# markods/GpuSeqAlign

Measured on AMD Instinct MI355X. Metric: GCUPS (DP cell updates/s) + peak HBM GB/s, NW-LG N×M fill, 1/2/4/8 MI355X, higher is better.
Workload: dtype int32; 1 GPU; BASELINE configs[2]: NW-LG 99899x100000 related pair, sparse tile-header (mlsp) fill, tileBx 256 x tileBy 1024, headers only in HBM; R=99899, C=100000, pairs_per_rank=1, representation=sparse tile headers (mlsp), parallelism=pair-sharded x1

## Files before the change

gpuseqalign_amd/__init__.py:

```python
from __future__ import annotations

import ctypes
import dataclasses
import os
from typing import Callable, Dict, Optional, Sequence, Tuple

import numpy as np

__all__ = [
    "NwStat", "NwError", "lib", "Engine", "AlignResult", "SparseResult", "PairDev",
    "NwAlgorithm", "get_nw_algorithm_map", "hash_full", "trace_full", "trace_sparse", "hash_sparse",
    "sparse_align_cost", "sparse_tile_by", "KNOB_NAMES", "LAUNCH_KINDS",
]

_PKG = os.path.dirname(os.path.abspath(__file__))
_SO = os.environ.get("GSA_LIB") or os.path.join(_PKG, "libgsa.so")
_LIB = None


class NwStat:
    success = 0
    helpMenuRequested = 1
    errorCudaGeneral = 2
    errorMemoryAllocation = 3
# ... 42 lines not shown
    def as_dict(self):
        return {"checked": int(self.checked), "mismatches": int(self.mismatches), "first": int(self.first)}


class MemStats(ctypes.Structure):
    _fields_ = [("glmem_peak_allocs", ctypes.c_int64), ("shmem_peak_allocs", ctypes.c_int64),
                ("locmem_peak_allocs", ctypes.c_int64), ("regmem_peak_allocs", ctypes.c_int64)]

    def as_dict(self):
        return {k: int(getattr(self, k)) for k, _ in self._fields_}


class FullTiming(ctypes.Structure):
    _fields_ = [("pass1_ms", ctypes.c_float), ("pass2_ms", ctypes.c_float),
                ("clock_ghz_median", ctypes.c_float), ("clock_ghz_mean", ctypes.c_float),
                ("workgroups", ctypes.c_int64), ("fused", ctypes.c_int32), ("groups", ctypes.c_int32)]


class LaunchInfo(ctypes.Structure):
    _fields_ = [("kind", ctypes.c_int32), ("ns", ctypes.c_int32), ("k", ctypes.c_int32), ("q8", ctypes.c_int32),
                ("q8_declined", ctypes.c_int32), ("staged", ctypes.c_int32), ("mlsppt", ctypes.c_int32),
                ("both_ends", ctypes.c_int32), ("npairs", ctypes.c_int32), ("pair_major", ctypes.c_int32),
                ("trace_band", ctypes.c_int32),
                ("tickets", ctypes.c_int64), ("band_tiles", ctypes.c_int64)]


LAUNCH_KINDS = ("none", "full_lane", "full_fused", "full_two_launch", "sparse_krow", "sparse_strip", "score_krow",
                "score_strip", "score_scan", "trace_sparse", "score_lanes")


class ScoreResult(ctypes.Structure):
    _fields_ = [("score", ctypes.c_int32), ("i_end", ctypes.c_int64), ("j_end", ctypes.c_int64),
                ("calc_kernel_ms", ctypes.c_float)]


class AlignDbResult(ctypes.Structure):
    _fields_ = [("score", ctypes.c_int32), ("status", ctypes.c_int32), ("i_start", ctypes.c_int64),
                ("j_start", ctypes.c_int64), ("i_end", ctypes.c_int64), ("j_end", ctypes.c_int64),
                ("cigar_off", ctypes.c_int64), ("cigar_len", ctypes.c_int64)]


class AlignDbInfo(ctypes.Structure):
    _fields_ = [("lane_hits", ctypes.c_int32), ("unsupported", ctypes.c_int32), ("chunks", ctypes.c_int32),
                ("tasks", ctypes.c_int64), ("code_bytes", ctypes.c_int64), ("fill_ms", ctypes.c_float),
                ("walk_ms", ctypes.c_float)]


# ... 1312 lines not shown
```

gpuseqalign_amd/csrc/gsa_capi.hip:

```cpp
#include <hip/hip_runtime.h>

#include <algorithm>
#include <chrono>
#include <cstdio>
#include <cstdlib>
#include <cstring>
#include <map>
#include <new>
#include <string>
#include <thread>
#include <vector>

#include "../../include/gsa.h"
#include "gsa_ctx.h"
#include "nw_check.h"
#include "nw_lane.h"
#include "nw_expand.h"
#include "nw_krow.h"
#include "nw_strip.h"
#include "nw_trace_dev.h"

namespace gsa {
int fold_moves(const unsigned char* moves, int64_t n, char* edit, int64_t cap, int64_t* edit_len, uint32_t* trace_hash);
}
// ... 13 lines not shown
namespace {

constexpr const char* kKnobNames[] = {
    "GSA_SPARSE_KERNEL", "GSA_KROW_K",      "GSA_KROW_NS",      "GSA_KROW_Q8",       "GSA_LANE_NS",
    "GSA_LANE_FEED",     "GSA_LANE_PAIR",   "GSA_FULL_KERNEL",  "GSA_FULL_FUSED",    "GSA_FULL_SPLIT",
    "GSA_FUSED_STAGED",
    "GSA_EXPAND_RR",     "GSA_BATCH_ORDER", "GSA_SCORE_SCAN",   "GSA_SCORE_KERNEL",  "GSA_SCORE_K",
    "GSA_SCORE_BIDI",    "GSA_SCORE_BIDI_SW", "GSA_BIDI_GRAN",  "GSA_BIDI_SKEW",     "GSA_BIDI_SW_CONT",
    "GSA_BIDI_LOG",      "GSA_TRACE_BAND",  "GSA_TRACE_BAND_BUDGET", "GSA_STAMPS",     "GSA_DB_LANES",
    "GSA_DB_MAXC"};

bool knob_known(const char* name)
{
    for (const char* k : kKnobNames)
        if (std::strcmp(k, name) == 0) return true;
    return false;
}

enum SparseKern { kSpStrip, kSpKrow };
SparseKern sparse_kernel(const gsa_ctx* ctx)
{
    const char* e = knob(ctx, "GSA_SPARSE_KERNEL");
    return (e && std::strcmp(e, "strip") == 0) ? kSpStrip : kSpKrow;
}



int lane_ns(const gsa_ctx* ctx)
{
    const char* e = knob(ctx, "GSA_LANE_NS");
    const int v = e ? std::atoi(e) : gsa::kLaneNSDefault;
    return ((v >= 1 && v <= 4) || v == 6 || v == 8) ? v : gsa::kLaneNSDefault;
}

int run_check(gsa_ctx* ctx, gsa::CheckArgs& a, bool sparse, hipStream_t st, gsa_check_result* out)
{
    hipError_t e = hipSetDevice(ctx->device);
    if (e != hipSuccess) return fail(ctx, e, GSA_ERROR_CUDA_GENERAL);
    int s = reserve_hard(ctx, ctx->buf[kBufChk], 64);
    if (s != GSA_SUCCESS) return s;
    unsigned long long* const chk = ctx->buf[kBufChk].as<unsigned long long>();
    const unsigned long long init[3] = {0ull, 0ull, ~0ull};
    unsigned long long res[3];
    if ((e = hipMemcpyAsync(chk, init, sizeof(init), hipMemcpyHostToDevice, st)) != hipSuccess)
        return fail(ctx, e, GSA_ERROR_MEMORY_TRANSFER);
    a.res = chk;
// ... 93 lines not shown
    for (int p = 0; p < npairs; ++p)
        tileRows += std::max<long long>(1, ((long long)pairs[p].adjrows - 1 + gsa::kSparseTileBy - 1) / gsa::kSparseTileBy);
    const bool fitsChip = tileRows <= (long long)std::max(1, ctx->cu_count);
    const int nsDefault = (npairs > 1 && !fitsChip) ? gsa::kKrowNSBatchDefault : gsa::kKrowNSDefault;
    int krowK = env_int(ctx, "GSA_KROW_K", gsa::kKrowKDefault), krowNS = env_int(ctx, "GSA_KROW_NS", nsDefault);
    if (rows64)
    {
        krowK = 4;
        krowNS = fused ? fused->ns : env_int(ctx, "GSA_KROW_NS", (npairs > 1 && !fitsChip) ? 8 : 4) == 8 ? 8 : 4;
    }
    if (!gsa::krow_ok(krowNS, krowK) || (done && gsa::krow_ticket_rows(krowNS, krowK) != gsa::kSparseTileBy))
    {
        krowK = gsa::kKrowKDefault;
        krowNS = gsa::kKrowNSDefault;
    }
    a.ns = lane ? lane_ns(ctx) : krow ? krowNS : gsa::kSparseNS;
    if (krow && env_int(ctx, "GSA_KROW_Q8", 1) != 0)
    {
        const size_t lds8 = fused ? gsa::full_fused_lds_bytes(krowNS, substsz, true, fused->staged)
                                  : gsa::krow_lds_bytes(krowNS, krowNS == 2 ? 512 : 1024, substsz, true);
        a.q8 = lds8 <= (size_t)ctx->lds_max ? 1 : 0;
    }
    a.q8flag = ctx->ctl + 2;
    const int fullRows = gsa::kLaneRows * a.ns;
    if (mode == gsa::kModeSparse)
    {
        if (tileBx < 64 || tileBx % 16 != 0) return GSA_ERROR_INVALID_VALUE;
        a.tBx = tileBx;
        a.tBy = gsa::kSparseTileBy;
    }
    std::vector<gsa::PairDesc> hd((size_t)npairs);
    long long tickets = 0, gran = 0, maxWork = 1, span = 1;
    for (int p = 0; p < npairs; ++p)
    {
        const gsa_pair_dev& in = pairs[p];
        if (in.adjrows < 1 || in.adjcols < 1 || !in.seqY || !in.seqX) return GSA_ERROR_INVALID_VALUE;
        gsa::PairDesc& d = hd[(size_t)p];
        std::memset(&d, 0, sizeof(d));
        d.seqY = in.seqY;
        d.seqX = in.seqX;
        d.R = in.adjrows - 1;
        d.C = in.adjcols - 1;
        if (mode == gsa::kModeFull)
        {
            if (!in.score) return GSA_ERROR_INVALID_VALUE;
            d.score = in.score;
// ... 32 lines not shown
        tickets += d.nTickets;
        gran += (long long)d.nTickets * gsa::gran_stride(d.Cp);
        if (tickets > (1ll << 30)) return GSA_ERROR_INVALID_VALUE;
    }
    const std::vector<int> sched = batch_schedule(ctx, hd, tickets);
    hipError_t e;
    int s = stage_descs(ctx, hd, sched, st);
    if (s != GSA_SUCCESS) return s;

    gsa::PairDesc* const ddesc = ctx->buf[kBufDesc].as<gsa::PairDesc>();
    a.pairs = ddesc;
    a.nPairs = npairs;
    a.nTicketsTotal = (int)tickets;
    a.sched = sched.empty() ? nullptr : (const int*)(ddesc + npairs);
    a.qcap = (int)(0x7fffffffll / span);
    e = gsa::launch_headers(a, mode, maxWork, st);
    if (e != hipSuccess) return fail(ctx, e, GSA_ERROR_KERNEL_FAILURE);
    auto record = [&](unsigned epoch) {
        gsa_launch_info& li = new_launch_info(
            ctx, lane ? GSA_LAUNCH_FULL_LANE : krow ? GSA_LAUNCH_SPARSE_KROW : GSA_LAUNCH_SPARSE_STRIP, st, epoch);
        li.ns = a.ns;
        li.k = krow ? krowK : 1;
        li.q8 = a.q8;
        li.mlsppt = done ? 1 : 0;
        li.npairs = npairs;
        li.pair_major = (npairs > 1 && sched.empty()) ? 1 : 0;
        li.tickets = tickets;
    };
    if (tickets == 0)
    {
        record(0);
        return GSA_SUCCESS;
    }

    if ((s = ensure_gran(ctx, (size_t)gran, st)) != GSA_SUCCESS) return s;
    a.gran = ctx->buf[kBufGran].as<unsigned long long>();
    a.ticket = ctx->ctl;
    a.err = ctx->ctl + 1;
    a.spin = ctx->spin_ticks;
    a.done = done;
    a.ptChunk = std::max(1, ptChunk);
    a.epoch = ++ctx->epoch;
    if (a.epoch == 0) a.epoch = ++ctx->epoch;
    if (fused)
    {
        if (!rows64) return GSA_ERROR_INVALID_VALUE;
// ... 9 lines not shown
            a.xP = fused->p1;
            a.xrole = ctx->ctl + 4;
            a.xcounter = ctx->ctl + 5;
            if ((e = hipMemsetAsync(a.xrole, 0, 8, st)) != hipSuccess) return fail(ctx, e, GSA_ERROR_MEMORY_TRANSFER);
            ctx->stamps_n = 0;
            if (env_int(ctx, "GSA_STAMPS", 0) &&
                (s = reserve_stamps(ctx, 4 * words + 3 * (size_t)a.xTasks, st, &a.stamps)) != GSA_SUCCESS)
                return s;
        }
        a.xdone = ctx->buf[kBufXdone].as<unsigned long long>();
    }
    if (!fused && krow && !lane && env_int(ctx, "GSA_STAMPS", 0))
    {
        if ((s = reserve_stamps(ctx, 10 * (size_t)tickets * (size_t)krowNS, st, &a.stamps)) != GSA_SUCCESS) return s;
    }
    e = hipMemsetAsync(ctx->ctl, 0, 4, st);
    if (e != hipSuccess) return fail(ctx, e, GSA_ERROR_MEMORY_TRANSFER);
    int grid = (npairs == 1) ? std::max(1, std::min((int)tickets, ctx->cu_count)) : 0;
    a.laneFeed = knob(ctx, "GSA_LANE_FEED") ? env_int(ctx, "GSA_LANE_FEED", 0) : -1;
    a.lanePair = knob(ctx, "GSA_LANE_PAIR") ? env_int(ctx, "GSA_LANE_PAIR", 0) : -1;
    e = lane     ? gsa::launch_lane_fill(a, a.ns, grid, st)
        : fused  ? gsa::launch_full_fused(a, fused->ns, fused->waves, fused->staged, 0, st)
        : rows64 ? gsa::launch_krow_fill_xr(a, krowNS, grid, st)
        : krow   ? gsa::launch_krow_fill(a, krowNS, krowK, 0, grid, st)
                 : gsa::launch_strip_fill(a, mode, grid, st);
    if (e != hipSuccess) return fail(ctx, e, GSA_ERROR_KERNEL_FAILURE);
    note_launch(ctx);
    record(a.epoch);
    return GSA_SUCCESS;
}

int enqueue_fill(gsa_ctx* ctx, int mode, const int32_t* seqY, int32_t adjrows, const int32_t* seqX, int32_t adjcols,
                 const int32_t* subst, int32_t substsz, int32_t gapo, int32_t* score, int32_t tileBx, int32_t* hrow,
                 int32_t* hcol, hipStream_t st, unsigned long long* done = nullptr, int ptChunk = 0,
                 const int32_t* ld = nullptr)
{
    gsa_pair_dev p {seqY, adjrows, seqX, adjcols, score, hrow, hcol};
    return enqueue_batch(ctx, mode, 1, &p, subst, substsz, gapo, tileBx, st, done, ptChunk, ld);
}

constexpr int kNoScratch = -1000;

struct TwoPassOpts
{
    int slot = 0;
    hipEvent_t afterP1 = nullptr, beforeP1 = nullptr, timeP1 = nullptr, startEv = nullptr;
    bool split = false;
// ... 1488 lines not shown
```

gpuseqalign_amd/csrc/nw_krow.h:

```cpp
#pragma once
#include <hip/hip_runtime.h>
#include <stddef.h>

#include "nw_strip.h"

namespace gsa {

constexpr int kKrowKDefault = 4;
constexpr int kKrowNSDefault = 4;
constexpr int kKrowNSBatchDefault = 8;

__host__ __device__ constexpr bool krow_ok(int ns, int k)
{
    return ((k == 2 || k == 4) && (ns == 2 || ns == 4)) || (k == 4 && ns == 8);
}
__host__ __device__ constexpr int krow_ticket_rows(int ns, int k) { return ns * 64 * k; }
__host__ __device__ constexpr int krow_tickets(int trows, int ns, int k)
{
    return (trows * kSparseTileBy + krow_ticket_rows(ns, k) - 1) / krow_ticket_rows(ns, k);
}
size_t krow_lds_bytes(int ns, int lw, int substsz, bool q8 = false);
hipError_t launch_krow_fill(const StripArgs& a, int ns, int k, int lw, int grid, hipStream_t stream);
hipError_t launch_krow_fill_xr(const StripArgs& a, int ns, int grid, hipStream_t stream);
size_t full_fused_lds_bytes(int ns, int substsz, bool q8, bool staged);
hipError_t launch_full_fused(const StripArgs& a, int ns, int waves, bool staged, int grid, hipStream_t stream);

size_t krow_score_lds_bytes(int substsz, bool q8 = false);
hipError_t launch_krow_score(const StripArgs& a, int mode, int k, int grid, hipStream_t stream);
hipError_t launch_krow_score_affine(const StripArgs& a, int mode, int k, int grid, hipStream_t stream);
hipError_t launch_krow_score_semi(const StripArgs& a, int mode, int k, int grid, hipStream_t stream);
hipError_t launch_semi_rowmax(const int* rowR, int R, int C, int go, int ge, int* score, int* jend, hipStream_t stream);
hipError_t launch_krow_score_overlap(const StripArgs& a, int mode, int k, int grid, hipStream_t stream);
hipError_t launch_overlap_max(const int* rowR, const int* colC, int R, int C, int go, int ge, int* res, hipStream_t stream);
hipError_t launch_krow_score_semi_batch(const StripArgs& a, int mode, int k, int grid, hipStream_t stream);
hipError_t launch_semi_rowmax_batch(const PairDesc* pairs, int nPairs, int go, int ge, const unsigned* err, ScoreOut* out,
                                    hipStream_t stream);
hipError_t launch_krow_score_overlap_batch(const StripArgs& a, int mode, int k, int grid, hipStream_t stream);
hipError_t launch_overlap_max_batch(const PairDesc* pairs, int nPairs, int go, int ge, const unsigned* err, ScoreOut* out,
                                    hipStream_t stream);

}
```

gpuseqalign_amd/csrc/nw_krow.hip:

```cpp
#ifndef GSA_PROBE_P1
#define GSA_PROBE_P1 0
#endif
#ifndef GSA_FX_VMCNT
#define GSA_FX_VMCNT 16
#endif
#include <hip/hip_runtime.h>
#include <stdint.h>

#include <algorithm>

#include "nw_expand.h"
#include "nw_krow.h"
#ifdef GSA_KROW_XR
#include "nw_expand_dev.h"
#endif

namespace gsa {
namespace {

__host__ __device__ constexpr int kr_qrs(int lw, bool q8 = false) { return (q8 ? lw / 4 : lw / 2) + 32; }
__host__ __device__ constexpr uint32_t kr_copy1(int lw, int substsz, bool q8 = false)
{
    return (uint32_t)substsz * kr_qrs(lw, q8) + (q8 ? 8u : 16u);
}
// ... 2 lines not shown
    return q8 ? 4u * kr_copy1(lw, substsz, true) : kr_copy1(lw, substsz) + (uint32_t)substsz * kr_qrs(lw) + 16u;
}
constexpr int kBlk = 16;
constexpr int kHalo = kBlk / 4;
constexpr int kRing = 512;
constexpr int kBig = 0x3fffffff;
constexpr int kSubRow = 36;
constexpr int kBatch = 128;
__host__ __device__ constexpr uint32_t kr_prog(int i) { return 8u * (uint32_t)i; }
__host__ __device__ constexpr uint32_t kr_cons(int i) { return 8u * (uint32_t)(i + 1) + 4u; }
constexpr uint32_t kFXo = 4, kFTicket = 132;
constexpr uint32_t kFCap = 160;
constexpr int kXD = 32;
constexpr int kLedgerWords = 10;
#ifndef GSA_KR_BLOCK_LEDGER
#define GSA_KR_BLOCK_LEDGER 0
#endif
#ifndef GSA_KR_LEDGER
#define GSA_KR_LEDGER GSA_KR_BLOCK_LEDGER
#endif
__host__ __device__ constexpr uint32_t kr_xwords(uint32_t flags) { return flags + 256u; }
__host__ __device__ constexpr uint32_t kr_xdata(uint32_t flags) { return flags + 256u + 64u; }
[[maybe_unused]] __host__ __device__ constexpr uint32_t kr_xstage_bytes(int ns) { return 64u + (uint32_t)ns * kXD * 256u; }

extern __shared__ __attribute__((aligned(16))) char krsm[];


typedef int int4v __attribute__((ext_vector_type(4)));
typedef int int2v __attribute__((ext_vector_type(2)));
template <typename T>
using gptr = __attribute__((address_space(1))) T*;
template <typename T>
__device__ __forceinline__ gptr<T> G(T* p)
{
    return (gptr<T>)p;
}

__device__ __forceinline__ int lds_ld(uint32_t a) { return *(const int*)(krsm + a); }
__device__ __forceinline__ void lds_st(uint32_t a, int v) { *(int*)(krsm + a) = v; }
__device__ __forceinline__ int4v lds_ld4(uint32_t a) { return *(const int4v*)(krsm + a); }
__device__ __forceinline__ int raw_ld(uint32_t a)
{
    return __hip_atomic_load((int*)__builtin_assume_aligned(krsm + a, 4), __ATOMIC_RELAXED, __HIP_MEMORY_SCOPE_WORKGROUP);
}
__device__ __forceinline__ int flag_ld(uint32_t a) { return __builtin_amdgcn_readfirstlane(raw_ld(a)); }
__device__ __forceinline__ void flag_st(uint32_t a, int v)
// ... 17 lines not shown
{
    int r;
    asm("v_cndmask_b32_e64 %0, %1, %2, %3" : "=v"(r) : "v"(a), "v"(b), "s"(m));
    return r;
}
__device__ __forceinline__ int qlo(int v) { return (int)(short)v; }
__device__ __forceinline__ int qhi(int v) { return v >> 16; }

struct KrLds
{
    uint32_t q, sub, ring, flags;
};

__host__ __device__ inline KrLds kr_layout(int ns, int lw, int substsz, bool q8 = false)
{
    KrLds L;
    L.q = 0;
    L.sub = kr_qdwords(lw, substsz, q8) * 4u;
    L.ring = L.sub + (uint32_t)substsz * kSubRow * 4u;
    L.flags = L.ring + (uint32_t)(ns + 1) * kRing * 4u;
    return L;
}

template <int NS, int K, int LW, int PT, bool Q8>
__device__ __forceinline__ void kr_strip(const StripArgs& a, const KrLds& L, int tk, int w, int lane)
{
    const int g = a.g;
    const int Cp = a.Cp;
    const int tBx = a.tBx, tBy = a.tBy, tcols = a.tcols;
    const int r0 = tk * (64 * K * NS) + 64 * K * w + 1;
    const int rl = r0 + K * lane;
    constexpr int kLW = LW, kQRS = kr_qrs(LW, Q8);
    constexpr int kQW = Q8 ? kLW / 4 : kLW / 2;
    constexpr int kQD = Q8 ? 4 : 8;
    uint32_t qrow[K];
#pragma unroll
    for (int k = 0; k < K; ++k)
    {
        const int r = rl + k;
        int y = (r <= a.R) ? G(a.seqY)[r] : 0;
        y = ((unsigned)y < (unsigned)a.substsz) ? y : 0;
        qrow[k] = L.q + 4u * ((uint32_t)(lane & (Q8 ? 3 : 1)) * kr_copy1(LW, a.substsz, Q8) + (uint32_t)y * kQRS);
    }
    const uint32_t ring_in = L.ring + (uint32_t)w * (kRing * 4u);
    const uint32_t ring_out = L.ring + (uint32_t)(w + 1) * (kRing * 4u);
    const uint32_t rbase = lane == 0 ? ring_in : ring_out;
    uint32_t roff = lane == 0 ? 4u * 64u : 0u;
    const uint32_t f_in = L.flags + kr_prog(w), f_out = L.flags + kr_prog(w + 1);
    const uint32_t c_out = L.flags + kr_cons(w + 1);
// ... 163 lines not shown
                "ds_write_b128 %7, %10 offset:32\n"
                "ds_write_b128 %7, %11 offset:48\n"
                "s_mov_b64 exec, 1\n"
                "ds_write_b32 %12, %13\n"
                "s_mov_b64 exec, %4\n"
                "s_waitcnt lgkmcnt(5)"
                : "+v"(hc[0]), "+v"(hc[1]), "+v"(hc[2]), "+v"(hc[3]), "=&s"(sv)
                : "v"(hb), "s"(K == 4 ? 0x8000800080008000ull : 0x8000000080000000ull), "v"(sa),
                  "v"(int4v {lt[0], lt[1], lt[2], lt[3]}), "v"(int4v {lt[4], lt[5], lt[6], lt[7]}),
                  "v"(int4v {lt[8], lt[9], lt[10], lt[11]}), "v"(int4v {lt[12], lt[13], lt[14], lt[15]}),
                  "v"(xsWords + 4u * (uint32_t)w), "v"(b)
                : "memory");
        }
        else
            halo_load(b);
    };
    int rpin = 0, rpco = 0, rpxo = 0;
    int rsink = 0;
    const int xoAdd = (w == 0) ? 64 + kBlk - 2 * kBlk : kBig;
    int nbb = tBx / kBlk, jb = 1;
    constexpr bool pt = PT == 1;
    constexpr bool fx = PT >= 3;
    int ptPend = 0;

    auto block = [&](int b, int (&qc)[K][kQD], int (&qn)[K][kQD], auto rampT, bool cap) {
        constexpr bool RAMP = decltype(rampT)::value;
        constexpr bool CAP = !RAMP;
#if GSA_KR_BLOCK_LEDGER
        const uint64_t lt0 = GSA_LDG_T();
        if (ldgEnd) ldg[3] += lt0 - ldgEnd;
#endif
        {
            const int slack = __builtin_amdgcn_readfirstlane(min(min(rpin, rpco + (64 + kRing)), rpxo + xoAdd));
            asm volatile("" ::"v"(rpin), "v"(rpco), "v"(rpxo), "v"(rsink));
            if (slack < kBlk * b + 64 + kBlk && !spin(b)) return false;
        }
        if (PT == 3 && b > 0)
            halo_stage(b);
        else
            halo_load(b);
#if GSA_KR_BLOCK_LEDGER
        const uint64_t lt1 = GSA_LDG_T();
#endif
        const uint32_t pn = q_off(b + 1);
        int va[CAP ? K : 1][CAP ? kBlk : 1];
#pragma unroll
        for (int u = 0; u < kBlk; ++u)
        {
            int nh[K];
            const int up = shr1z(H[K - 1]) + hc[u >> 2][u & 3];
            nh[0] = max3i(D + qv(qc, 0, u), up, H[0]);
#pragma unroll
            for (int k = 1; k < K; ++k) nh[k] = max3i(H[k - 1] + qv(qc, k, u), nh[k - 1], H[k]);
            if constexpr (RAMP)
            {
                const bool border = lane >= kBlk * b + u;
#pragma unroll
                for (int k = 0; k < K; ++k) nh[k] = border ? 0 : nh[k];
            }
            if (u < kQD)
#pragma unroll
                for (int k = 0; k < K; ++k) qn[k][u] = lds_ld(qrow[k] + pn + 4u * u);
            lt[u] = H[K - 1];
            D = up;
#pragma unroll
            for (int k = 0; k < K; ++k)
            {
                H[k] = nh[k];
                if constexpr (CAP) va[k][u] = nh[k];
            }
            if (u == kBlk - 2)
            {
                asm volatile("" ::: "memory");
                const int2v lo = *(const int2v*)(krsm + f_in), hi = *(const int2v*)(krsm + f_in + 16u);
                asm volatile("" ::: "memory");
                rpin = lo.x;
                rpxo = lo.y;
                rpco = hi.y;
                rsink = hi.x;
            }
        }
#if GSA_KR_BLOCK_LEDGER
        const uint64_t lt2 = GSA_LDG_T();
#endif
        handoff(b);
        roff = (roff + 4u * kBlk) & (4u * kRing - 1);
        if constexpr (PT == 4 && !RAMP)
            if ((b & 15) == 15)
            {
                asm volatile("s_waitcnt vmcnt(16)" ::: "memory");
                if (lane == 0)
                    __hip_atomic_store(a.xdone + (size_t)tk * NS + w,
                                       ((unsigned long long)a.epoch << 32) | (unsigned)max(0, kBlk * (b - 7)),
                                       __ATOMIC_RELAXED, __HIP_MEMORY_SCOPE_AGENT);
            }
        if constexpr (PT == 3 && !RAMP)
            if ((b & 15) == 15)
            {
                asm volatile("s_waitcnt vmcnt(%0)" ::"n"(8 * K) : "memory");
                flag_st(xsWords + 4u * (uint32_t)(2 * NS + w), max(0, kBlk * (b + 1) - 2 * tBx - 64));
                const uint64_t t0 = __builtin_amdgcn_s_memrealtime();
                for (unsigned it = 1; flag_ld(xsWords + 4u * (uint32_t)(NS + w)) + kXD < b + 1 + 16; ++it)
                {
                    __builtin_amdgcn_s_sleep(1);
                    if (__builtin_amdgcn_s_memrealtime() - t0 > a.spin || ((it & 31) == 0 && err_set(a)))
                    {
                        atomicOr(a.err, 1u);
                        return false;
                    }
                }
            }
        if (CAP && cap)
        {
            if (pt && ptPend)
            {
                asm volatile("s_waitcnt vmcnt(0)" ::: "memory");
                flag_st(L.flags + kFCap + 4u * (uint32_t)w, ptPend);
                ptPend = 0;
            }
            constexpr uint64_t m1 = 0xAAAAAAAAAAAAAAAAull, m2 = 0xCCCCCCCCCCCCCCCCull;
            constexpr uint64_t m4 = 0xF0F0F0F0F0F0F0F0ull, m8 = 0xFF00FF00FF00FF00ull;
            int v[K];
#pragma unroll
            for (int k = 0; k < K; ++k)
            {
                int x[8];
#pragma unroll
                for (int i = 0; i < 8; ++i) x[i] = sel(m1, va[k][2 * i], va[k][2 * i + 1]);
#pragma unroll
                for (int i = 0; i < 4; ++i) x[i] = sel(m2, x[2 * i], x[2 * i + 1]);
#pragma unroll
                for (int i = 0; i < 2; ++i) x[i] = sel(m4, x[2 * i], x[2 * i + 1]);
                v[k] = sel(m8, x[0], x[1]);
            }
            const int gb = (rl + kBlk * nbb) * g;
// ... 663 lines not shown
                                           __HIP_MEMORY_SCOPE_AGENT);
                    pub[w] = x;
                    moved = true;
                }
                all = all && pub[w] == (int)kXDone;
            }
            if (all) return;
        }
        const uint64_t now = __builtin_amdgcn_s_memrealtime();
        if (moved)
            last = now;
        else
        {
            if (now - last > 4 * a.spin || ((idle & 63) == 0 && err_set(a)))
            {
                atomicOr(a.err, 1u);
                return;
            }
            __builtin_amdgcn_s_sleep(1);
        }
    }
}

__device__ __forceinline__ PairDesc kr_desc(const PairDesc* p)
{
    constexpr int N = sizeof(PairDesc) / 4;
    const int* wds = (const int*)p;
    union
    {
        int v[N];
        PairDesc d;
    } u;
#pragma unroll
    for (int k = 0; k < N; ++k) u.v[k] = __builtin_amdgcn_readfirstlane(G(wds)[k]);
    return u.d;
}

template <int NS, int PT = 0>
constexpr bool kr_split() { return NS <= 4; }
template <int NS, int PT = 0>
constexpr int kr_waves() { return NS + 2 + (kr_split<NS, PT>() ? 1 : 0); }

template <int NS, int K, int LW, int PT, bool Q8>
__global__ void __launch_bounds__((64 * kr_waves<NS, PT>()), 1) nw_krow_kernel(StripArgs a)
{
    const int w = __builtin_amdgcn_readfirstlane(threadIdx.x >> 6);
// ... 75 lines not shown
        else if (kr_split<NS, PT>() && w == NS + 2)
            kr_loader<NS, K, LW, 2, Q8>(pa, L, tk, lane);
        else
        {
            unsigned long long* const lg = (GSA_KR_LEDGER && a.stamps) ? a.stamps + kLedgerWords * ((size_t)tkg * NS + w) : nullptr;
            pa.stamps = lg ? a.stamps + kLedgerWords * (size_t)tkg * NS : nullptr;
            if (lg && lane == 0)
            {
                lg[0] = __builtin_amdgcn_s_memrealtime();
                lg[2] = __builtin_amdgcn_s_memtime();
            }
            __builtin_amdgcn_s_setprio(3);
            kr_strip<NS, K, LW, PT, Q8>(pa, L, tk, w, lane);
            __builtin_amdgcn_s_setprio(0);
            if (lg && lane == 0)
            {
                lg[1] = __builtin_amdgcn_s_memrealtime();
                lg[3] = __builtin_amdgcn_s_memtime();
            }
        }
    }
}

template <int NS, int K, int LW, int PT, bool Q8>
hipError_t launch_kr1(const StripArgs& a, int grid, hipStream_t stream, bool foot = true)
{
    const size_t lds = krow_lds_bytes(NS, LW, a.substsz, Q8);
    auto kern = nw_krow_kernel<NS, K, LW, PT, Q8>;
    hipError_t e = hipFuncSetAttribute((const void*)kern, hipFuncAttributeMaxDynamicSharedMemorySize, (int)lds);
    if (e != hipSuccess) return e;
    if (grid <= 0)
    {
        int per_cu = 0, dev = 0, cus = 0;
        e = hipOccupancyMaxActiveBlocksPerMultiprocessor(&per_cu, (const void*)kern, 64 * kr_waves<NS, PT>(), lds);
        if (e == hipSuccess) e = hipGetDevice(&dev);
        if (e == hipSuccess) e = hipDeviceGetAttribute(&cus, hipDeviceAttributeMultiprocessorCount, dev);
        if (e != hipSuccess) return e;
        grid = std::max(1, std::min(a.nTicketsTotal, std::max(1, per_cu) * cus));
    }
    if (foot && (e = record_foot((const void*)kern, lds, 64 * kr_waves<NS, PT>(), grid)) != hipSuccess) return e;
    hipLaunchKernelGGL(kern, dim3(grid), dim3(64 * kr_waves<NS, PT>()), lds, stream, a);
    return hipGetLastError();
}

template <int NS, int K, int LW, int PT = 0>
hipError_t launch_kr(const StripArgs& a, int grid, hipStream_t stream)
{
    if (!a.q8) return launch_kr1<NS, K, LW, PT, false>(a, grid, stream);
    hipError_t e = launch_kr1<NS, K, LW, PT, true>(a, grid, stream);
    if (e != hipSuccess) return e;
    StripArgs b = a;
    b.q8 = 2;
    return launch_kr1<NS, K, LW, PT, false>(b, grid, stream, false);
}

#ifdef GSA_KROW_SCORE
constexpr int kNegS = -(1 << 29);
typedef int int4u __attribute__((ext_vector_type(4), aligned(4)));
typedef int int2u __attribute__((ext_vector_type(2), aligned(4)));
__device__ __forceinline__ int ks_sel(int a, int b, uint64_t m)
{
    int r;
    asm("v_cndmask_b32_e64 %0, %1, %2, %3" : "=v"(r) : "v"(a), "v"(b), "s"(m));
    return r;
}
__device__ __forceinline__ void ks_sel0(int (&r)[2], const int (&a)[2], const int (&b)[2], int x)
{
    asm("v_cmp_eq_u32 vcc, 0, %6\n\tv_cndmask_b32 %0, %2, %4, vcc\n\tv_cndmask_b32 %1, %3, %5, vcc"
        : "=&v"(r[0]), "=&v"(r[1])
        : "v"(a[0]), "v"(a[1]), "v"(b[0]), "v"(b[1]), "v"(x)
        : "vcc");
}
__device__ __forceinline__ void ks_sel0(int (&r)[4], const int (&a)[4], const int (&b)[4], int x)
{
    asm("v_cmp_eq_u32 vcc, 0, %12\n\tv_cndmask_b32 %0, %4, %8, vcc\n\tv_cndmask_b32 %1, %5, %9, vcc\n\t"
        "v_cndmask_b32 %2, %6, %10, vcc\n\tv_cndmask_b32 %3, %7, %11, vcc"
// ... 1345 lines not shown
{
    if (!a.q8) return launch_fused1<NS, W, false, PTF>(a, grid, stream, true);
    hipError_t e = launch_fused1<NS, W, true, PTF>(a, grid, stream, true);
    if (e != hipSuccess) return e;
    StripArgs b = a;
    b.q8 = 2;
    return launch_fused1<NS, W, false, PTF>(b, grid, stream, false);
}

}

size_t full_fused_lds_bytes(int ns, int substsz, bool q8, bool staged)
{
    return std::max(krow_lds_bytes(ns, 1024, substsz, q8) + (staged ? kr_xstage_bytes(ns) : 0u), expand_stream_lds_bytes(substsz));
}

hipError_t launch_full_fused(const StripArgs& a, int ns, int waves, bool staged, int grid, hipStream_t stream)
{
    if (!a.xpair || !a.xdone || !a.xrole || !a.xcounter) return hipErrorInvalidValue;
    if (ns == 4 && waves == 8) return staged ? launch_fused<4, 8, 3>(a, grid, stream) : launch_fused<4, 8, 4>(a, grid, stream);
    return hipErrorInvalidValue;
}
#elif defined(GSA_KROW_BATCH8)
hipError_t launch_krow_fill_b8(const StripArgs& a, int grid, hipStream_t stream)
{
    return launch_kr<8, 4, 1024>(a, grid, stream);
}
#else
hipError_t launch_krow_fill_b8(const StripArgs& a, int grid, hipStream_t stream);

size_t krow_lds_bytes(int ns, int lw, int substsz, bool q8) { return (size_t)kr_layout(ns, lw, substsz, q8).flags + 256; }

hipError_t launch_krow_fill(const StripArgs& a, int ns, int k, int lw, int grid, hipStream_t stream)
{
    if (k == 2) return ns == 2 ? launch_kr<2, 2, 512>(a, grid, stream) : launch_kr<4, 2, 1024>(a, grid, stream);
    (void)lw;
    if (ns == 8) return launch_krow_fill_b8(a, grid, stream);
    if (a.done) return launch_kr<4, 4, 1024, 1>(a, grid, stream);
    return ns == 2 ? launch_kr<2, 4, 512>(a, grid, stream) : launch_kr<4, 4, 1024>(a, grid, stream);
}
#endif

}
```

include/gsa.h:

```cpp
#ifndef GSA_H
#define GSA_H

#include <stdint.h>

#ifdef __cplusplus
extern "C" {
#endif

enum gsa_stat
{
    GSA_SUCCESS = 0,
    GSA_HELP_MENU_REQUESTED = 1,
    GSA_ERROR_CUDA_GENERAL = 2,
    GSA_ERROR_MEMORY_ALLOCATION = 3,
    GSA_ERROR_MEMORY_TRANSFER = 4,
    GSA_ERROR_KERNEL_FAILURE = 5,
    GSA_ERROR_IO_STREAM = 6,
    GSA_ERROR_INVALID_FORMAT = 7,
    GSA_ERROR_INVALID_VALUE = 8,
    GSA_ERROR_INVALID_RESULT = 9
};

typedef struct gsa_ctx gsa_ctx;

// ... 93 lines not shown
    GSA_LAUNCH_FULL_TWO_LAUNCH = 3,
    GSA_LAUNCH_SPARSE_KROW = 4,
    GSA_LAUNCH_SPARSE_STRIP = 5,
    GSA_LAUNCH_SCORE_KROW = 6,
    GSA_LAUNCH_SCORE_STRIP = 7,
    GSA_LAUNCH_SCORE_SCAN = 8,
    GSA_LAUNCH_TRACE_SPARSE = 9,
    GSA_LAUNCH_SCORE_LANES = 10
};
typedef struct gsa_launch_info
{
    int32_t kind;
    int32_t ns, k;
    int32_t q8;
    int32_t q8_declined;
    int32_t staged;
    int32_t mlsppt;
    int32_t both_ends;
    int32_t npairs;
    int32_t pair_major;
    int32_t trace_band;
    int64_t tickets;
    int64_t band_tiles;
} gsa_launch_info;
int gsa_last_launch(gsa_ctx* ctx, gsa_launch_info* out);

uint32_t gsa_hash_full(const int32_t* score, int32_t adjrows, int32_t adjcols);
int gsa_trace_full(const int32_t* score, const int32_t* seqY, int32_t adjrows, const int32_t* seqX,
                   int32_t adjcols, char* edit, int64_t cap, int64_t* edit_len, uint32_t* trace_hash);
int gsa_trace_sparse(const int32_t* tileHrowMat, const int32_t* tileHcolMat, const gsa_sparse_geom* geom,
                     const int32_t* seqY, int32_t adjrows, const int32_t* seqX, int32_t adjcols,
                     const int32_t* subst, int32_t substsz, int32_t gapo, char* edit, int64_t cap,
                     int64_t* edit_len, uint32_t* trace_hash, int32_t* align_cost);
uint32_t gsa_hash_sparse(const int32_t* tileHrowMat, const int32_t* tileHcolMat, const gsa_sparse_geom* geom,
                         const int32_t* seqY, int32_t adjrows, const int32_t* seqX, int32_t adjcols,
                         const int32_t* subst, int32_t substsz, int32_t gapo);
int32_t gsa_sparse_align_cost(const int32_t* tileHrowMat, const int32_t* tileHcolMat, const gsa_sparse_geom* geom,
                              const int32_t* seqY, int32_t adjrows, const int32_t* seqX, int32_t adjcols,
                              const int32_t* subst, int32_t substsz, int32_t gapo);

typedef struct gsa_check_result
{
    int64_t checked;
    int64_t mismatches;
    int64_t first;
} gsa_check_result;
// ... 258 lines not shown
```

Before: 2016 GCUPS.

## Park tile-column headers in LDS and drain them via a dedicated column wave

New measurement: 1643 GCUPS. -18.5%, worse.

```diff
diff --git a/gpuseqalign_amd/__init__.py b/gpuseqalign_amd/__init__.py
--- a/gpuseqalign_amd/__init__.py
+++ b/gpuseqalign_amd/__init__.py
@@ -88,7 +88,8 @@
                 ("q8_declined", ctypes.c_int32), ("staged", ctypes.c_int32), ("mlsppt", ctypes.c_int32),
                 ("both_ends", ctypes.c_int32), ("npairs", ctypes.c_int32), ("pair_major", ctypes.c_int32),
                 ("trace_band", ctypes.c_int32),
-                ("tickets", ctypes.c_int64), ("band_tiles", ctypes.c_int64)]
+                ("tickets", ctypes.c_int64), ("band_tiles", ctypes.c_int64),
+                ("park", ctypes.c_int32), ("reserved0", ctypes.c_int32)]
 
 
 LAUNCH_KINDS = ("none", "full_lane", "full_fused", "full_two_launch", "sparse_krow", "sparse_strip", "score_krow",
diff --git a/gpuseqalign_amd/csrc/gsa_capi.hip b/gpuseqalign_amd/csrc/gsa_capi.hip
--- a/gpuseqalign_amd/csrc/gsa_capi.hip
+++ b/gpuseqalign_amd/csrc/gsa_capi.hip
@@ -59,6 +59,11 @@
 {
     const char* e = knob(ctx, "GSA_SPARSE_KERNEL");
     return (e && std::strcmp(e, "strip") == 0) ? kSpStrip : kSpKrow;
+}
+bool sparse_park(const gsa_ctx* ctx)
+{
+    const char* e = knob(ctx, "GSA_SPARSE_KERNEL");
+    return !(e && std::strcmp(e, "krow-tree") == 0);
 }
 
 
@@ -198,6 +203,9 @@
         a.q8 = lds8 <= (size_t)ctx->lds_max ? 1 : 0;
     }
     a.q8flag = ctx->ctl + 2;
+    const bool park = krow && !lane && !done && !rows64 && !fused && krowK == 4 && (krowNS == 4 || krowNS == 8) &&
+                      sparse_park(ctx) && gsa::krow_park_lds_bytes(krowNS, substsz, false) <= (size_t)ctx->lds_max &&
+                      (!a.q8 || gsa::krow_park_lds_bytes(krowNS, substsz, true) <= (size_t)ctx->lds_max);
     const int fullRows = gsa::kLaneRows * a.ns;
     if (mode == gsa::kModeSparse)
     {
@@ -276,6 +284,7 @@
         li.ns = a.ns;
         li.k = krow ? krowK : 1;
         li.q8 = a.q8;
+        li.park = park ? 1 : 0;
         li.mlsppt = done ? 1 : 0;
         li.npairs = npairs;
         li.pair_major = (npairs > 1 && sched.empty()) ? 1 : 0;
@@ -331,7 +340,7 @@
     e = lane     ? gsa::launch_lane_fill(a, a.ns, grid, st)
         : fused  ? gsa::launch_full_fused(a, fused->ns, fused->waves, fused->staged, 0, st)
         : rows64 ? gsa::launch_krow_fill_xr(a, krowNS, grid, st)
-        : krow   ? gsa::launch_krow_fill(a, krowNS, krowK, 0, grid, st)
+        : krow   ? gsa::launch_krow_fill(a, krowNS, krowK, 0, park, grid, st)
                  : gsa::launch_strip_fill(a, mode, grid, st);
     if (e != hipSuccess) return fail(ctx, e, GSA_ERROR_KERNEL_FAILURE);
     note_launch(ctx);
diff --git a/gpuseqalign_amd/csrc/nw_krow.h b/gpuseqalign_amd/csrc/nw_krow.h
--- a/gpuseqalign_amd/csrc/nw_krow.h
+++ b/gpuseqalign_amd/csrc/nw_krow.h
@@ -20,7 +20,8 @@
     return (trows * kSparseTileBy + krow_ticket_rows(ns, k) - 1) / krow_ticket_rows(ns, k);
 }
 size_t krow_lds_bytes(int ns, int lw, int substsz, bool q8 = false);
-hipError_t launch_krow_fill(const StripArgs& a, int ns, int k, int lw, int grid, hipStream_t stream);
+size_t krow_park_lds_bytes(int ns, int substsz, bool q8);
+hipError_t launch_krow_fill(const StripArgs& a, int ns, int k, int lw, bool park, int grid, hipStream_t stream);
 hipError_t launch_krow_fill_xr(const StripArgs& a, int ns, int grid, hipStream_t stream);
 size_t full_fused_lds_bytes(int ns, int substsz, bool q8, bool staged);
 hipError_t launch_full_fused(const StripArgs& a, int ns, int waves, bool staged, int grid, hipStream_t stream);
diff --git a/gpuseqalign_amd/csrc/nw_krow.hip b/gpuseqalign_amd/csrc/nw_krow.hip
--- a/gpuseqalign_amd/csrc/nw_krow.hip
+++ b/gpuseqalign_amd/csrc/nw_krow.hip
@@ -48,6 +48,10 @@
 __host__ __device__ constexpr uint32_t kr_xwords(uint32_t flags) { return flags + 256u; }
 __host__ __device__ constexpr uint32_t kr_xdata(uint32_t flags) { return flags + 256u + 64u; }
 [[maybe_unused]] __host__ __device__ constexpr uint32_t kr_xstage_bytes(int ns) { return 64u + (uint32_t)ns * kXD * 256u; }
+__host__ __device__ constexpr uint32_t kr_pwords(uint32_t flags) { return flags + 256u; }
+__host__ __device__ constexpr uint32_t kr_pdata(uint32_t flags) { return flags + 256u + 64u; }
+constexpr uint32_t kParkSlot = 64u * 16u;
+[[maybe_unused]] __host__ __device__ constexpr uint32_t kr_park_bytes(int ns) { return 64u + (uint32_t)ns * 2u * kParkSlot; }
 
 extern __shared__ __attribute__((aligned(16))) char krsm[];
 
@@ -111,9 +115,10 @@
     return L;
 }
 
-template <int NS, int K, int LW, int PT, bool Q8>
+template <int NS, int K, int LW, int PT, bool Q8, bool PARK = false>
 __device__ __forceinline__ void kr_strip(const StripArgs& a, const KrLds& L, int tk, int w, int lane)
 {
+    static_assert(!PARK || (PT == 0 && K == 4), "parking: plain fills, a 16-byte quad per lane");
     const int g = a.g;
     const int Cp = a.Cp;
     const int tBx = a.tBx, tBy = a.tBy, tcols = a.tcols;
@@ -323,6 +328,16 @@
     constexpr bool pt = PT == 1;
     constexpr bool fx = PT >= 3;
     int ptPend = 0;
+    [[maybe_unused]] uint32_t parkA, parkD, parkW;
+    [[maybe_unused]] int pk[PARK ? K : 1][PARK ? kBlk : 1];
+    [[maybe_unused]] uint64_t parkM = 0;
+    [[maybe_unused]] uint32_t parkP = 0;
+    if constexpr (PARK)
+    {
+        parkA = kr_pdata(L.flags) + (uint32_t)(2 * w + 1) * kParkSlot + 16u * (uint32_t)lane;
+        parkD = 0u - kParkSlot;
+        parkW = kr_pwords(L.flags) + 4u * (uint32_t)w;
+    }
 
     auto block = [&](int b, int (&qc)[K][kQD], int (&qn)[K][kQD], auto rampT, bool cap) {
         constexpr bool RAMP = decltype(rampT)::value;
@@ -343,8 +358,58 @@
 #if GSA_KR_BLOCK_LEDGER
         const uint64_t lt1 = GSA_LDG_T();
 #endif
+        if constexpr (CAP && PARK)
+        {
+            if (parkM != 0)
+            {
+                uint64_t sv;
+#define GSA_PARK_Q(u) "v"(int4v {pk[0][u], pk[1][u], pk[2][u], pk[3][u]})
+                asm volatile(
+                    "s_mov_b64 %0, exec\n"
+                    "s_mov_b64 exec, %1\n"
+                    "ds_write_b128 %2, %3\n"
+                    "s_lshl_b64 exec, exec, 1\n"
+                    "ds_write_b128 %2, %4\n"
+                    "s_lshl_b64 exec, exec, 1\n"
+                    "ds_write_b128 %2, %5\n"
+                    "s_lshl_b64 exec, exec, 1\n"
+                    "ds_write_b128 %2, %6\n"
+                    "s_lshl_b64 exec, exec, 1\n"
+                    "ds_write_b128 %2, %7\n"
+                    "s_lshl_b64 exec, exec, 1\n"
+                    "ds_write_b128 %2, %8\n"
+                    "s_lshl_b64 exec, exec, 1\n"
+                    "ds_write_b128 %2, %9\n"
+                    "s_lshl_b64 exec, exec, 1\n"
+                    "ds_write_b128 %2, %10\n"
+                    "s_lshl_b64 exec, exec, 1\n"
+                    "ds_write_b128 %2, %11\n"
+                    "s_lshl_b64 exec, exec, 1\n"
+                    "ds_write_b128 %2, %12\n"
+                    "s_lshl_b64 exec, exec, 1\n"
+                    "ds_write_b128 %2, %13\n"
+                    "s_lshl_b64 exec, exec, 1\n"
+                    "ds_write_b128 %2, %14\n"
+                    "s_lshl_b64 exec, exec, 1\n"
+                    "ds_write_b128 %2, %15\n"
+                    "s_lshl_b64 exec, exec, 1\n"
+                    "ds_write_b128 %2, %16\n"
+                    "s_lshl_b64 exec, exec, 1\n"
+                    "ds_write_b128 %2, %17\n"
+                    "s_lshl_b64 exec, exec, 1\n"
+                    "ds_write_b128 %2, %18\n"
+                    "s_mov_b64 exec, %0"
+                    : "=&s"(sv)
+                    : "s"(parkM), "v"(parkP), GSA_PARK_Q(0), GSA_PARK_Q(1), GSA_PARK_Q(2), GSA_PARK_Q(3),
+                      GSA_PARK_Q(4), GSA_PARK_Q(5), GSA_PARK_Q(6), GSA_PARK_Q(7), GSA_PARK_Q(8), GSA_PARK_Q(9),
+                      GSA_PARK_Q(10), GSA_PARK_Q(11), GSA_PARK_Q(12), GSA_PARK_Q(13), GSA_PARK_Q(14), GSA_PARK_Q(15)
+                    : "memory", "scc");
+#undef GSA_PARK_Q
+                parkM = 0;
+            }
+        }
         const uint32_t pn = q_off(b + 1);
-        int va[CAP ? K : 1][CAP ? kBlk : 1];
+        int va[(CAP && !PARK) ? K : 1][(CAP && !PARK) ? kBlk : 1];
 #pragma unroll
         for (int u = 0; u < kBlk; ++u)
         {
@@ -368,7 +433,10 @@
             for (int k = 0; k < K; ++k)
             {
                 H[k] = nh[k];
-                if constexpr (CAP) va[k][u] = nh[k];
+                if constexpr (CAP && PARK)
+                    pk[k][u] = nh[k];
+                else if constexpr (CAP)
+                    va[k][u] = nh[k];
             }
             if (u == kBlk - 2)
             {
@@ -411,7 +479,35 @@
                     }
                 }
             }
-        if (CAP && cap)
+        if constexpr (CAP && PARK)
+        {
+            if (cap)
+            {
+                if (b == nbb && jb > 2 && flag_ld(parkW) < jb - 2)
+                {
+                    const uint64_t t0 = __builtin_amdgcn_s_memrealtime();
+                    for (unsigned it = 1; flag_ld(parkW) < jb - 2; ++it)
+                    {
+                        __builtin_amdgcn_s_sleep(1);
+                        if (__builtin_amdgcn_s_memrealtime() - t0 > a.spin || ((it & 31) == 0 && err_set(a)))
+                        {
+                            atomicOr(a.err, 1u);
+                            return false;
+                        }
+                    }
+                }
+                parkM = 1ull << (kBlk * (b - nbb));
+                parkP = parkA;
+                if (b == nbb + 3)
+                {
+                    nbb += tBx / kBlk;
+                    ++jb;
+                    parkA += parkD;
+                    parkD = 0u - parkD;
+                }
+            }
+        }
+        else if (CAP && cap)
         {
             if (pt && ptPend)
             {
@@ -1121,6 +1217,62 @@
     }
 }
 
+template <int NS, int K>
+__device__ __forceinline__ void kr_column(const StripArgs& a, const KrLds& L, int tk, int lane)
+{
+    static_assert(K == 4, "a 16-byte quad per lane");
+    const int g = a.g, tBx = a.tBx, tBy = a.tBy, tcols = a.tcols;
+    const uint32_t W = kr_pwords(L.flags), D = kr_pdata(L.flags) + 16u * (uint32_t)lane;
+    int jb[NS];
+    uint32_t gb[NS];
+    size_t hoff[NS];
+    bool fin = true;
+#pragma unroll
+    for (int w = 0; w < NS; ++w)
+    {
+        const int r0 = tk * (64 * K * NS) + 64 * K * w + 1, rl = r0 + K * lane;
+        const bool capRows = 64 * K * NS <= kSparseTileBy || (r0 - 1) / tBy < a.trows;
+        const int iT = (rl - 1) / tBy;
+        jb[w] = capRows ? 1 : tcols;
+        gb[w] = (uint32_t)rl * (uint32_t)g;
+        hoff[w] = (size_t)iT * (size_t)tcols * (size_t)(tBy + 1) + (size_t)(rl - iT * tBy);
+        fin = fin && jb[w] >= tcols;
+    }
+    uint64_t last = __builtin_amdgcn_s_memrealtime();
+    for (unsigned idle = 1; !fin; ++idle)
+    {
+        bool moved = false;
+        fin = true;
+#pragma unroll
+        for (int w = 0; w < NS; ++w)
+        {
+            if (jb[w] < tcols && flag_ld(L.flags + kr_prog(w + 1)) >= jb[w] * tBx + 5 * kBlk)
+            {
+                const int4v v = lds_ld4(D + (uint32_t)(2 * w + (jb[w] & 1)) * kParkSlot);
+                flag_st(W + 4u * (uint32_t)w, jb[w]);
+                const gptr<int> p = G(a.hcol) + hoff[w] + (size_t)jb[w] * (size_t)(tBy + 1);
+                const uint32_t gc = gb[w] + (uint32_t)(jb[w] * tBx) * (uint32_t)g;
+#pragma unroll
+                for (int k = 0; k < K; ++k) p[k] = (int)((uint32_t)v[k] + gc + (uint32_t)k * (uint32_t)g);
+                ++jb[w];
+                moved = true;
+            }
+            fin = fin && jb[w] >= tcols;
+        }
+        if (moved)
+            last = __builtin_amdgcn_s_memrealtime();
+        else
+        {
+            if (__builtin_amdgcn_s_memrealtime() - last > 4 * a.spin || ((idle & 63) == 0 && err_set(a)))
+            {
+                atomicOr(a.err, 1u);
+                return;
+            }
+            __builtin_amdgcn_s_sleep(16);
+        }
+    }
+}
+
 __device__ __forceinline__ PairDesc kr_desc(const PairDesc* p)
 {
     constexpr int N = sizeof(PairDesc) / 4;
@@ -1242,36 +1394,148 @@
     }
 }
 
-template <int NS, int K, int LW, int PT, bool Q8>
+template <int NS, int K, int LW, bool Q8>
+__global__ void __launch_bounds__((64 * (kr_waves<NS, 0>() + 1)), 1) nw_krow_park_kernel(StripArgs a)
+{
+    constexpr int PT = 0;
+    constexpr int kThreads = 64 * (kr_waves<NS, PT>() + 1);
+    const int w = __builtin_amdgcn_readfirstlane(threadIdx.x >> 6);
+    const int lane = threadIdx.x & 63;
+    const KrLds L = kr_layout(NS, LW, a.substsz, Q8);
+    if (!Q8 && a.q8 == 2 && __hip_atomic_load(a.q8flag, __ATOMIC_RELAXED, __HIP_MEMORY_SCOPE_AGENT) != a.epoch) return;
+    bool bad = false, bad8 = false;
+    for (int k = threadIdx.x; k < a.substsz * kSubRow; k += kThreads)
+    {
+        const int x = k / kSubRow, yy = k % kSubRow;
+        const int v = yy < a.substsz ? G(a.subst)[yy * a.substsz + x] - 2 * a.g : 0;
+        bad |= v < -32768 || v > 32767 || v > a.qcap;
+        bad8 |= v < -128 || v > 127 || v > a.qcap;
+        lds_st(L.sub + 4u * k, v);
+    }
+    if constexpr (Q8)
+    {
+        if (threadIdx.x == 0) lds_st(L.flags + kFTicket, 0);
+        __syncthreads();
+        if (bad8) atomicOr((int*)(krsm + L.flags + kFTicket), 1);
+        __syncthreads();
+        if (lds_ld(L.flags + kFTicket) != 0)
+        {
+            if (threadIdx.x == 0) __hip_atomic_store(a.q8flag, a.epoch, __ATOMIC_RELAXED, __HIP_MEMORY_SCOPE_AGENT);
+            return;
+        }
+    }
+    else if (bad)
+        atomicOr(a.err, 2u);
+    for (;;)
+    {
+        __syncthreads();
+        if (threadIdx.x == 0) lds_st(L.flags + kFTicket, err_set(a) ? a.nTicketsTotal : (int)atomicAdd(a.ticket, 1u));
+        __syncthreads();
+        const int tkg = __builtin_amdgcn_readfirstlane(lds_ld(L.flags + kFTicket));
+        if (tkg >= a.nTicketsTotal) break;
+        int lo = 0, tks = -1;
+        if (a.sched)
+        {
+            lo = __builtin_amdgcn_readfirstlane(G(a.sched)[2 * tkg]);
+            tks = __builtin_amdgcn_readfirstlane(G(a.sched)[2 * tkg + 1]);
+        }
+        else
+        {
+            int hi = a.nPairs - 1;
+            while (lo < hi)
+            {
+                const int mid = (lo + hi + 1) >> 1;
+                if (__builtin_amdgcn_readfirstlane(G(a.pairs)[mid].ticketBase) <= tkg)
+                    lo = mid;
+                else
+                    hi = mid - 1;
+            }
+        }
+        const PairDesc d = kr_desc(a.pairs + lo);
+        StripArgs pa = a;
+        pa.seqY = d.seqY;
+        pa.seqX = d.seqX;
+        pa.R = d.R;
+        pa.C = d.C;
+        pa.Cp = d.Cp;
+        pa.nTickets = d.nTickets;
+        pa.hrow = d.hrow;
+        pa.hcol = d.hcol;
+        pa.trows = d.trows;
+        pa.tcols = d.tcols;
+        pa.gran = a.gran + d.granOff;
+        pa.granStride = gran_stride(d.Cp);
+        pa.rows64 = d.rows64;
+        pa.rpitch = d.rpitch;
+        const int tk = (tks >= 0) ? tks : tkg - d.ticketBase;
+        if (threadIdx.x < 32) lds_st(L.flags + 4u * threadIdx.x, 0);
+        if (threadIdx.x >= kFCap / 4 && threadIdx.x < kFCap / 4 + 8) lds_st(L.flags + 4u * threadIdx.x, 0);
+        if (threadIdx.x >= 64 && threadIdx.x < 64 + NS) lds_st(kr_pwords(L.flags) + 4u * (threadIdx.x - 64), 0);
+        __syncthreads();
+        if (w == kr_waves<NS, PT>())
+            kr_column<NS, K>(pa, L, tk, lane);
+        else if (w == NS + 1)
+            kr_drain<NS, K, LW, PT>(pa, L, tk, lane);
+        else if (w == NS)
+            kr_loader<NS, K, LW, kr_split<NS, PT>() ? 1 : 0, Q8, true>(pa, L, tk, lane);
+        else if (kr_split<NS, PT>() && w == NS + 2)
+            kr_loader<NS, K, LW, 2, Q8>(pa, L, tk, lane);
+        else
+        {
+            unsigned long long* const lg = (GSA_KR_LEDGER && a.stamps) ? a.stamps + kLedgerWords * ((size_t)tkg * NS + w) : nullptr;
+            pa.stamps = lg ? a.stamps + kLedgerWords * (size_t)tkg * NS : nullptr;
+            if (lg && lane == 0)
+            {
+                lg[0] = __builtin_amdgcn_s_memrealtime();
+                lg[2] = __builtin_amdgcn_s_memtime();
+            }
+            __builtin_amdgcn_s_setprio(3);
+            kr_strip<NS, K, LW, PT, Q8, true>(pa, L, tk, w, lane);
+            __builtin_amdgcn_s_setprio(0);
+            if (lg && lane == 0)
+            {
+                lg[1] = __builtin_amdgcn_s_memrealtime();
+                lg[3] = __builtin_amdgcn_s_memtime();
+            }
+        }
+    }
+}
+
+template <int NS, int K, int LW, int PT, bool Q8, bool PARK = false>
 hipError_t launch_kr1(const StripArgs& a, int grid, hipStream_t stream, bool foot = true)
 {
-    const size_t lds = krow_lds_bytes(NS, LW, a.substsz, Q8);
-    auto kern = nw_krow_kernel<NS, K, LW, PT, Q8>;
+    const size_t lds = krow_lds_bytes(NS, LW, a.substsz, Q8) + (PARK ? kr_park_bytes(NS) : 0u);
+    constexpr int kThreads = 64 * (kr_waves<NS, PT>() + (PARK ? 1 : 0));
+    void (*kern)(StripArgs);
+    if constexpr (PARK)
+        kern = nw_krow_park_kernel<NS, K, LW, Q8>;
+    else
+        kern = nw_krow_kernel<NS, K, LW, PT, Q8>;
     hipError_t e = hipFuncSetAttribute((const void*)kern, hipFuncAttributeMaxDynamicSharedMemorySize, (int)lds);
     if (e != hipSuccess) return e;
     if (grid <= 0)
     {
         int per_cu = 0, dev = 0, cus = 0;
-        e = hipOccupancyMaxActiveBlocksPerMultiprocessor(&per_cu, (const void*)kern, 64 * kr_waves<NS, PT>(), lds);
+        e = hipOccupancyMaxActiveBlocksPerMultiprocessor(&per_cu, (const void*)kern, kThreads, lds);
         if (e == hipSuccess) e = hipGetDevice(&dev);
         if (e == hipSuccess) e = hipDeviceGetAttribute(&cus, hipDeviceAttributeMultiprocessorCount, dev);
         if (e != hipSuccess) return e;
         grid = std::max(1, std::min(a.nTicketsTotal, std::max(1, per_cu) * cus));
     }
-    if (foot && (e = record_foot((const void*)kern, lds, 64 * kr_waves<NS, PT>(), grid)) != hipSuccess) return e;
-    hipLaunchKernelGGL(kern, dim3(grid), dim3(64 * kr_waves<NS, PT>()), lds, stream, a);
+    if (foot && (e = record_foot((const void*)kern, lds, kThreads, grid)) != hipSuccess) return e;
+    hipLaunchKernelGGL(kern, dim3(grid), dim3(kThreads), lds, stream, a);
     return hipGetLastError();
 }
 
-template <int NS, int K, int LW, int PT = 0>
+template <int NS, int K, int LW, int PT = 0, bool PARK = false>
 hipError_t launch_kr(const StripArgs& a, int grid, hipStream_t stream)
 {
-    if (!a.q8) return launch_kr1<NS, K, LW, PT, false>(a, grid, stream);
-    hipError_t e = launch_kr1<NS, K, LW, PT, true>(a, grid, stream);
+    if (!a.q8) return launch_kr1<NS, K, LW, PT, false, PARK>(a, grid, stream);
+    hipError_t e = launch_kr1<NS, K, LW, PT, true, PARK>(a, grid, stream);
     if (e != hipSuccess) return e;
     StripArgs b = a;
     b.q8 = 2;
-    return launch_kr1<NS, K, LW, PT, false>(b, grid, stream, false);
+    return launch_kr1<NS, K, LW, PT, false, PARK>(b, grid, stream, false);
 }
 
 #ifdef GSA_KROW_SCORE
@@ -2663,21 +2927,25 @@
     return hipErrorInvalidValue;
 }
 #elif defined(GSA_KROW_BATCH8)
-hipError_t launch_krow_fill_b8(const StripArgs& a, int grid, hipStream_t stream)
-{
-    return launch_kr<8, 4, 1024>(a, grid, stream);
+hipError_t launch_krow_fill_b8(const StripArgs& a, bool park, int grid, hipStream_t stream)
+{
+    return park ? launch_kr<8, 4, 1024, 0, true>(a, grid, stream) : launch_kr<8, 4, 1024>(a, grid, stream);
 }
 #else
-hipError_t launch_krow_fill_b8(const StripArgs& a, int grid, hipStream_t stream);
+hipError_t launch_krow_fill_b8(const StripArgs& a, bool park, int grid, hipStream_t stream);
 
 size_t krow_lds_bytes(int ns, int lw, int substsz, bool q8) { return (size_t)kr_layout(ns, lw, substsz, q8).flags + 256; }
 
-hipError_t launch_krow_fill(const StripArgs& a, int ns, int k, int lw, int grid, hipStream_t stream)
-{
+size_t krow_park_lds_bytes(int ns, int substsz, bool q8) { return krow_lds_bytes(ns, 1024, substsz, q8) + kr_park_bytes(ns); }
+
+hipError_t launch_krow_fill(const StripArgs& a, int ns, int k, int lw, bool park, int grid, hipStream_t stream)
+{
+    if (park && (k != 4 || (ns != 4 && ns != 8) || a.done)) return hipErrorInvalidValue;
     if (k == 2) return ns == 2 ? launch_kr<2, 2, 512>(a, grid, stream) : launch_kr<4, 2, 1024>(a, grid, stream);
     (void)lw;
-    if (ns == 8) return launch_krow_fill_b8(a, grid, stream);
+    if (ns == 8) return launch_krow_fill_b8(a, park, grid, stream);
     if (a.done) return launch_kr<4, 4, 1024, 1>(a, grid, stream);
+    if (park) return launch_kr<4, 4, 1024, 0, true>(a, grid, stream);
     return ns == 2 ? launch_kr<2, 4, 512>(a, grid, stream) : launch_kr<4, 4, 1024>(a, grid, stream);
 }
 #endif
diff --git a/include/gsa.h b/include/gsa.h
--- a/include/gsa.h
+++ b/include/gsa.h
@@ -139,6 +139,8 @@
     int32_t trace_band;
     int64_t tickets;
     int64_t band_tiles;
+    int32_t park;
+    int32_t reserved0;
 } gsa_launch_info;
 int gsa_last_launch(gsa_ctx* ctx, gsa_launch_info* out);
 
```
